# guzba/zippy

Hardware: NVIDIA H100
Metric: compress_level1_gzip_input_throughput (higher is better)
Workload: dtype u8

## Files before the change

zippy_b200/csrc/zb_deflate.cu:

```cuda
#include "zb_device.cuh"
#include "zb_kernels.h"
#include "zb_huff_warp.cuh"

#define LZ_THREADS (ZB_WARPS_PER_CHUNK * 32)
#define LZ_HASH_BITS 11
#define LZ_TABLE_ENTRIES (1 << LZ_HASH_BITS)
#define LZ_PRESEED 2048
#ifndef ZB_LZ1_RESOLVE_WINNER
#define ZB_LZ1_RESOLVE_WINNER 0
#endif
#define LZ_LANE_CAP 32

#define LZ_PIECE_BYTES ZB_REC_PIECE_BYTES
#define LZ_PHASES (ZB_SUB_BYTES / LZ_PIECE_BYTES)
#define LZ_PHASE_BYTES (ZB_CHUNK_BYTES / LZ_PHASES)
#define LZ_PHASE_HIST 1024
#define LZ_BATCH_LPW 2
#define LZ_BATCH_WINDOWS (32 / LZ_BATCH_LPW)
static_assert(LZ_PIECE_BYTES * ZB_WARPS_PER_CHUNK == LZ_PHASE_BYTES, "one piece per warp and phase");
static_assert(LZ_PIECE_BYTES / ZB_WINDOW % LZ_BATCH_WINDOWS == 0, "a batch of windows never straddles two pieces");

#define LZ_SM_DATA 0
#define LZ_SM_DATA_BYTES (LZ_PHASE_BYTES + LZ_PHASE_HIST + 64 + 384)
#define LZ_SM_TABLE (LZ_SM_DATA + LZ_SM_DATA_BYTES)
#define LZ_SM_TABLE_BYTES (ZB_WARPS_PER_CHUNK * LZ_TABLE_ENTRIES * 2)
#define LZ_SM_HIST (LZ_SM_TABLE + LZ_SM_TABLE_BYTES)
#define LZ_SM_HIST_BYTES (ZB_WARPS_PER_CHUNK * ZB_HIST_WORDS * 4)
#define LZ_SM_RING (LZ_SM_HIST + LZ_SM_HIST_BYTES)
#define LZ_SM_RING_BYTES (ZB_WARPS_PER_CHUNK * LZ_BATCH_WINDOWS * ZB_MATCH_SLOTS * 4)
#define LZ_SM_LMUL (LZ_SM_RING + LZ_SM_RING_BYTES)
#define LZ_LMUL_PIECE 33
#define LZ_LMUL_PQ 49
#define LZ_SM_LMUL_BYTES (56 * 4)
#define LZ_SM_PART (LZ_SM_LMUL + LZ_SM_LMUL_BYTES)
#define LZ_SM_PART_BYTES (ZB_WARPS_PER_CHUNK * 24)
#define LZ_SM_BAR (LZ_SM_PART + LZ_SM_PART_BYTES)
#define LZ_SM_TOTAL (LZ_SM_BAR + 16)
static_assert(LZ_TABLE_ENTRIES * 2 >= 4096, "a warp's table region must hold the CRC step table");
static_assert(3 * (LZ_SM_TOTAL + 1024) <= 233472, "three CTAs per SM");
static_assert(LZ_SM_PART % 8 == 0 && LZ_SM_TABLE % 16 == 0, "alignment");

__device__ __forceinline__ uint32_t lz_hash(uint32_t v) { return (v * 0x9E3779B1u) >> (32 - LZ_HASH_BITS); }
__device__ __forceinline__ uint32_t shl_clamp(uint32_t x, uint32_t n) {
  uint32_t r;
  asm("shl.b32 %0, %1, %2;" : "=r"(r) : "r"(x), "r"(n));
  return r;
}
__device__ __forceinline__ uint32_t low_mask(uint32_t n) { return shl_clamp(1u, n) - 1u; }

__device__ __forceinline__ uint32_t lz_final_rec(uint32_t mlen, uint32_t dist, int &lc, int &dc) {
  uint32_t le, de;
  lc = (int)zb_len_code_bf(mlen, le);
  dc = (int)zb_dist_code_bf(dist, de);
  return (uint32_t)lc | (le << 5) | ((uint32_t)dc << 10) | (de << 15);
}


__device__ __forceinline__ void lz_select(const uint8_t *data, uint32_t off0, uint32_t wb, uint32_t b1, uint32_t cur,
                                          uint32_t nvalid, uint32_t &m, uint32_t dist, uint32_t *ring_slot,
                                          uint32_t &sel, uint32_t &ism, uint32_t &endw) {
  const int lane = zb_lane();
  const uint32_t mm = __ballot_sync(ZB_FULL, m != 0);
  endw = 0;
  ism = 0;
  if (mm) {
    const uint32_t lbit = 1u << lane;
    const uint32_t endp = (uint32_t)lane + m;
    const uint32_t rest = shl_clamp(1u, endp) ? (mm >> endp) : 0u;
    uint32_t nc = rest ? endp + (uint32_t)(__ffs((int)rest) - 1) : 32u;
    uint32_t vis = 1u << (cur + (uint32_t)(__ffs((int)(mm >> cur)) - 1));
#pragma unroll
    for (int r = 0; r < 3; r++) {
      vis |= __reduce_or_sync(ZB_FULL, (vis & lbit) ? shl_clamp(1u, nc) : 0u);
      const uint32_t t = __shfl_sync(ZB_FULL, nc, (int)(nc & 31u));
      nc = nc < 32u ? t : 32u;
    }
    ism = vis;
    const int lastm = 31 - __clz((int)ism);
    const uint32_t cov = (ism & lbit) ? (low_mask(endp) & ~low_mask((uint32_t)lane)) : 0u;
    const uint32_t covered = __reduce_or_sync(ZB_FULL, cov);
    uint32_t mlast = __shfl_sync(ZB_FULL, m, lastm);
    if (mlast >= LZ_LANE_CAP) {
      const uint32_t md = __shfl_sync(ZB_FULL, dist, lastm);
      const uint32_t pos = wb + (uint32_t)lastm;
      const uint32_t off = off0 + pos + LZ_LANE_CAP + 8u * (uint32_t)lane;
      uint32_t x0 = zb_ld32_unaligned(data, off) ^ zb_ld32_unaligned(data, off - md);
      uint32_t x1 = zb_ld32_unaligned(data, off + 4) ^ zb_ld32_unaligned(data, off + 4 - md);
      uint32_t nm = x0 ? ((uint32_t)(__ffs((int)x0) - 1) >> 3) : 4u + (x1 ? ((uint32_t)(__ffs((int)x1) - 1) >> 3) : 4u);
      uint32_t stop = __ballot_sync(ZB_FULL, nm < 8u);
      if (stop) {
        int first = __ffs((int)stop) - 1;
        mlast = LZ_LANE_CAP + 8u * (uint32_t)first + __shfl_sync(ZB_FULL, nm, first);
      } else {
        mlast = LZ_LANE_CAP + 256u;
      }
      mlast = min(mlast, min((uint32_t)ZB_MAX_MATCH, b1 - pos));
      if (lane == lastm) m = mlast;
    }
    sel = ism | (~covered & ~low_mask(cur) & low_mask(nvalid));
    endw = (uint32_t)lastm + mlast;
    if (ism & lbit) {
      uint32_t rank = (uint32_t)__popc(ism & (lbit - 1u));
      ring_slot[rank] = (m - 3u) | ((dist - 1u) << 9);
    }
  } else {
    sel = low_mask(nvalid) & ~low_mask(cur);
  }
}

template <int LPW, bool LITS>
__device__ __forceinline__ void lz_batch_pass(const uint8_t *wdata, bool active, uint32_t ksel, uint32_t kism,
                                              const uint32_t *ring_win, uint32_t *whist, uint2 *gmask_w,
                                              uint32_t *grecs_piece, uint32_t &rec_base) {
  constexpr int NW = 32 / LPW;
  const uint32_t part = (uint32_t)zb_lane() / NW, wi = (uint32_t)zb_lane() % NW;
  if (active && part == 0) *gmask_w = make_uint2(ksel, kism);
  const uint32_t im = active ? kism : 0u;
  const uint32_t pm = (0xffffffffu >> (32 - 32 / LPW)) << (part * (32 / LPW));
  uint32_t s = (LITS && active) ? (ksel & ~kism & pm) : 0u;
  while (s) {
    const uint32_t bit = (uint32_t)(__ffs((int)s) - 1);
    s &= s - 1;
    const uint32_t sy = wdata[bit];
    atomicAdd(&whist[sy >> 1], 1u << ((sy & 1u) * 16u));
  }
  const uint32_t nmatch = (uint32_t)__popc(im);
  uint32_t incl = nmatch;
#pragma unroll
  for (int o = 1; o < NW; o <<= 1) {
    const uint32_t t = __shfl_up_sync(ZB_FULL, incl, o, NW);
    if (wi >= (uint32_t)o) incl += t;
  }
  uint32_t *grecs_w = grecs_piece + rec_base + incl - nmatch;
  rec_base += __shfl_sync(ZB_FULL, incl, NW - 1);
  for (uint32_t k = part; k < nmatch; k += LPW) {
    const uint32_t raw = ring_win[k];
    int lc, dc;
    const uint32_t fin = lz_final_rec((raw & 511u) + 3u, (raw >> 9) + 1u, lc, dc);
    grecs_w[k] = fin;
    const uint32_t s1 = 257u + (uint32_t)lc, s2 = (uint32_t)ZB_NUM_LITLEN + (uint32_t)dc;
    atomicAdd(&whist[s1 >> 1], 1u << ((s1 & 1u) * 16u));
    atomicAdd(&whist[s2 >> 1], 1u << ((s2 & 1u) * 16u));
  }
}

#ifndef ZB_LZ1_STAGE_CLOCKS
#define ZB_LZ1_STAGE_CLOCKS 0
#endif
enum { LZS_WAIT, LZS_CHECKSUM, LZS_SEED, LZS_PROBE, LZS_EXTEND, LZS_SELECT, LZS_BATCH, LZS_BARRIER, LZS_N };
#if ZB_LZ1_STAGE_CLOCKS
__device__ unsigned long long zb_lz1_stage_clk[LZS_N];
#define LZ_CLK_DECL                          \
  unsigned long long clk_acc[LZS_N] = {};    \
  long long clk_t = clock64();
#define LZ_CLK(s)                            \
  if (MODE == 1) {                           \
    const long long clk_n = clock64();       \
    clk_acc[s] += (unsigned long long)(clk_n - clk_t); \
    clk_t = clk_n;                           \
  }
#define LZ_CLK_PUBLISH()                                                                           \
  if (MODE == 1 && lane == 0) {                                                                    \
    _Pragma("unroll") for (int s_ = 0; s_ < LZS_N; s_++) atomicAdd(&zb_lz1_stage_clk[s_], clk_acc[s_]); \
  }
extern "C" int zb200_lz1_stage_clocks(unsigned long long *out) {
  unsigned long long zero[LZS_N] = {};
  if (cudaMemcpyFromSymbol(out, zb_lz1_stage_clk, sizeof(zero)) != cudaSuccess) return -1;
  return cudaMemcpyToSymbol(zb_lz1_stage_clk, zero, sizeof(zero)) == cudaSuccess ? 0 : -1;
}
#else
#define LZ_CLK_DECL
#define LZ_CLK(s)
#define LZ_CLK_PUBLISH()
#endif

template <int MODE, int CK>
__global__ void __launch_bounds__(LZ_THREADS, 3)
    k_lz(const uint8_t *__restrict__ src, const ZbChunkDesc *__restrict__ desc, uint2 *__restrict__ masks,
         uint32_t *__restrict__ recs, uint16_t *__restrict__ hist, ZbChunkCheck *__restrict__ chk,
         const ZbCrcTables *__restrict__ tabs) {
  extern __shared__ __align__(128) uint8_t smem[];
  uint8_t *data = smem + LZ_SM_DATA;
  uint16_t *table_all = reinterpret_cast<uint16_t *>(smem + LZ_SM_TABLE);
  uint32_t *hist_all = reinterpret_cast<uint32_t *>(smem + LZ_SM_HIST);
  uint32_t *ring_all = reinterpret_cast<uint32_t *>(smem + LZ_SM_RING);
  uint32_t *lane_mul = reinterpret_cast<uint32_t *>(smem + LZ_SM_LMUL);
  uint64_t *part = reinterpret_cast<uint64_t *>(smem + LZ_SM_PART);
  uint64_t *bar = reinterpret_cast<uint64_t *>(smem + LZ_SM_BAR);

  const uint32_t chunk = blockIdx.x;
  const ZbChunkDesc d = desc[chunk];
  const uint32_t len = d.len;
  const int tid = (int)threadIdx.x, lane = tid & 31;
  const int warp = (int)__reduce_max_sync(ZB_FULL, (uint32_t)tid >> 5);

  if (tid == 0) {
    zb_mbar_init(bar, 1);
    zb_fence_mbar_init();
  }
  __syncthreads();
  const uint32_t mis = (uint32_t)((uintptr_t)(src + d.src_off) & 15u);

  uint16_t *table = table_all + warp * LZ_TABLE_ENTRIES;
  uint32_t *ring = ring_all + warp * LZ_BATCH_WINDOWS * ZB_MATCH_SLOTS;
  uint2 *gmask = masks + (size_t)chunk * ZB_WINDOWS_PER_CHUNK;
  uint32_t acc_crc = 0;
  uint64_t acc_a = 0, acc_b = 0;
  LZ_CLK_DECL

  for (uint32_t ph = 0; ph < LZ_PHASES; ph++) {
    const uint32_t pbase = ph * LZ_PHASE_BYTES;
    if (ph && pbase >= len) break;
    const uint32_t sbase = ph ? pbase - LZ_PHASE_HIST : 0u;
    if (ph) __syncthreads();
    LZ_CLK(LZS_BARRIER)
    if (tid == 0 && len) {
      zb_fence_proxy_async();
      zb_stage_chunk(data, src + d.src_off + sbase, min(len, pbase + LZ_PHASE_BYTES + 384u) - sbase, bar);
    }
    if (CK & ZB_CK_CRC) {
      uint32_t *crc_tab = reinterpret_cast<uint32_t *>(table);
      for (int i = lane; i < 1024; i += 32) crc_tab[i] = (&tabs->mul1024[0][0])[i];
    }
    if (ph == 0) {
      for (int i = tid; i < ZB_WARPS_PER_CHUNK * ZB_HIST_WORDS; i += LZ_THREADS) hist_all[i] = 0;
      if (tid < 33) lane_mul[tid] = tabs->lane_mul[tid];
      if (tid >= 64 && tid < 80) lane_mul[LZ_LMUL_PIECE + tid - 64] = tabs->piece_mul[tid - 64];
      if (tid >= 96 && tid < 100) lane_mul[LZ_LMUL_PQ + tid - 96] = tabs->pq_mul[tid - 96];
      __syncthreads();
    } else {
      __syncwarp();
    }
    if (len) zb_mbar_wait(bar, ph & 1u);
    LZ_CLK(LZS_WAIT)

    const uint32_t b0 = pbase + (uint32_t)warp * LZ_PIECE_BYTES;
    if (b0 >= len) continue;
    const uint32_t b1 = min(b0 + LZ_PIECE_BYTES, len);
    const uint32_t doff = mis - sbase;
    uint32_t *whist = hist_all + (b0 / ZB_SUB_BYTES) * ZB_HIST_WORDS;

    if (CK) {
      ZbCheck c = zb_warp_checksums<LZ_PIECE_BYTES, LZ_LMUL_PQ, CK>(data, doff + b0, b1 - b0,
                                                                    reinterpret_cast<const uint32_t *>(table), lane_mul);
      const uint32_t after = len - b1;
      if (after) {
        if (CK & ZB_CK_CRC) {
          const uint32_t shift = ((after & (LZ_PIECE_BYTES - 1)) == 0) ? lane_mul[LZ_LMUL_PIECE + after / LZ_PIECE_BYTES]
                                                                       : zb_xpow8_t(tabs->pow2, after);
          c.crc_raw = zb_gf2_mul(c.crc_raw, shift);
        }
        if (CK & ZB_CK_ADLER) c.b_sum += (uint64_t)after * c.a_sum;
      }
      acc_crc ^= c.crc_raw;
      acc_a += c.a_sum;
      acc_b += c.b_sum;
      __syncwarp();
    }
    LZ_CLK(LZS_CHECKSUM)

    if (MODE == 1) {
      uint4 ff = make_uint4(~0u, ~0u, ~0u, ~0u);
      uint4 *t4 = reinterpret_cast<uint4 *>(table);
      for (int i = lane; i < LZ_TABLE_ENTRIES * 2 / 16; i += 32) t4[i] = ff;
      __syncwarp();
      for (uint32_t s = b0 - min((uint32_t)LZ_PRESEED, b0 - sbase); s < b0; s += 32) {
        const uint32_t p = s + (uint32_t)lane;
        const bool can = p + 4 <= len;
        const uint32_t h = lz_hash(zb_ld32_unaligned(data, doff + p));
        if (can) table[h] = (uint16_t)p;
#if ZB_LZ1_RESOLVE_WINNER
        __syncwarp();
        for (;;) {
          const bool lost = can && table[h] < (uint16_t)p;
          if (!__any_sync(ZB_FULL, lost)) break;
          if (lost) table[h] = (uint16_t)p;
          __syncwarp();
        }
#endif
      }
      __syncwarp();
    }
    LZ_CLK(LZS_SEED)
    uint32_t entry = b0;
    uint32_t ksel = 0, kism = 0;
    uint32_t *grecs = recs + (size_t)chunk * ZB_RECS_PER_CHUNK + (b0 >> 2);
    uint32_t rec_base = 0;
    const uint32_t bl = (uint32_t)lane & (LZ_BATCH_WINDOWS - 1u);
    for (uint32_t wb = b0; wb < b1; wb += 32) {
      const uint32_t win = wb >> 5, slot = win & (LZ_BATCH_WINDOWS - 1u);
      uint32_t sel = 0, ism = 0;
      if (entry < wb + 32) {
        const uint32_t p = wb + (uint32_t)lane;
        const uint32_t nvalid = min(32u, b1 - wb);
        const uint32_t cur = entry - wb;
        uint32_t m = 0, c = 0, lit = 0;
        if (MODE == 1) {
          const uint32_t *wp = reinterpret_cast<const uint32_t *>(data) + ((doff + p) >> 2);
          const uint32_t sp = ((doff + p) & 3u) * 8u;
          const uint32_t p0 = wp[0], p1 = wp[1];
          const uint32_t v = __funnelshift_r(p0, p1, sp);
          lit = v & 255u;
          const bool can = (p + 4 <= len);
          const uint32_t h = lz_hash(v);
          c = table[h];
          __syncwarp();
          if (can) table[h] = (uint16_t)p;
#if ZB_LZ1_RESOLVE_WINNER
          __syncwarp();
          for (;;) {
            const bool lost = can && table[h] < (uint16_t)p;
            if (!__any_sync(ZB_FULL, lost)) break;
            if (lost) table[h] = (uint16_t)p;
            __syncwarp();
          }
#endif
          LZ_CLK(LZS_PROBE)
          const uint32_t limit = p < b1 ? min((uint32_t)ZB_MAX_MATCH, b1 - p) : 0u;
          if (can && c < p && p - c <= ZB_MAX_DIST && p >= entry && limit >= ZB_MIN_MATCH) {
            const uint32_t *wc = reinterpret_cast<const uint32_t *>(data) + ((doff + c) >> 2);
            const uint32_t sc = ((doff + c) & 3u) * 8u;
            uint32_t hp = p1, hc = wc[1];
            uint32_t np = wp[2], nq = wc[2], np2 = wp[3], nq2 = wc[3];
            if (__funnelshift_r(wc[0], hc, sc) == v) {
              m = 4;
#pragma unroll 1
              for (int k = 2;; k += 2) {
                const uint32_t x = __funnelshift_r(hp, np, sp) ^ __funnelshift_r(hc, nq, sc);
                const uint32_t x2 = __funnelshift_r(np, np2, sp) ^ __funnelshift_r(nq, nq2, sc);
                if (x) {
                  m += (uint32_t)(__ffs((int)x) - 1) >> 3;
                  break;
                }
                if (k == LZ_LANE_CAP / 4) {
                  m += 4;
                  break;
                }
                if (x2) {
                  m += 4u + ((uint32_t)(__ffs((int)x2) - 1) >> 3);
                  break;
                }
                m += 8;
                hp = np2;
                hc = nq2;
                np = wp[k + 2];
                nq = wc[k + 2];
                np2 = wp[k + 3];
                nq2 = wc[k + 3];
              }
              if (m < LZ_LANE_CAP) m = min(m, limit);
            }
          }
          LZ_CLK(LZS_EXTEND)
        }
        uint32_t endw;
        lz_select(data, doff, wb, b1, cur, nvalid, m, p - c, ring + slot * ZB_MATCH_SLOTS, sel, ism, endw);
        entry = wb + max(endw, nvalid);
        if (MODE == 1 && ((sel & ~ism) >> lane & 1u)) atomicAdd(&whist[lit >> 1], 1u << ((lit & 1u) * 16u));
        LZ_CLK(LZS_SELECT)
      }
      if (bl == slot) {
        ksel = sel;
        kism = ism;
      }
      if (slot == LZ_BATCH_WINDOWS - 1u || wb + 32 >= b1) {
        __syncwarp();
        const uint32_t bwin = win - slot + bl;
        lz_batch_pass<LZ_BATCH_LPW, MODE != 1>(data + (uint32_t)(doff + (bwin << 5)), bl <= slot, ksel, kism, ring + bl * ZB_MATCH_SLOTS,
                                    whist, gmask + bwin, grecs, rec_base);
        ksel = kism = 0;
        __syncwarp();
      }
      LZ_CLK(LZS_BATCH)
    }
  }
  if (lane == 0) {
    part[warp * 3 + 0] = acc_crc;
    part[warp * 3 + 1] = acc_a;
    part[warp * 3 + 2] = acc_b;
  }
  __syncthreads();
  {
    uint32_t *gh = reinterpret_cast<uint32_t *>(hist + (size_t)chunk * ZB_WARPS_PER_CHUNK * ZB_HIST_SYMS);
    for (int i = tid; i < ZB_WARPS_PER_CHUNK * ZB_HIST_WORDS; i += LZ_THREADS) gh[i] = hist_all[i];
  }
  LZ_CLK(LZS_BARRIER)
  LZ_CLK_PUBLISH()
  if (tid == 0) {
    uint32_t raw = 0;
    uint64_t a = 0, b = 0;
    for (int w = 0; w < ZB_WARPS_PER_CHUNK; w++) {
      raw ^= (uint32_t)part[w * 3 + 0];
      a += part[w * 3 + 1];
      b += part[w * 3 + 2];
    }
    ZbChunkCheck cc;
    cc.crc_raw = raw;
    cc.adler = (CK & ZB_CK_ADLER) ? zb_adler_from_sums(a % ZB_ADLER_MOD, b % ZB_ADLER_MOD, len) : 0u;
    chk[chunk] = cc;
  }
}

#define LZ2_HIST 32768
#define LZ2_SEG_BYTES ZB_SUB_BYTES
#define LZ2_SEGS ((ZB_CHUNK_BYTES + LZ2_HIST) / LZ2_SEG_BYTES)
#define LZ2_BUCKET_BITS 11
#define LZ2_BUCKETS (1 << LZ2_BUCKET_BITS)
#define LZ2_TABLES_PER_CTA (ZB_WARPS_PER_CHUNK + LZ2_SEGS)
#define LZ2_RING_WINDOWS 8
#define LZ2_SM_DATA_BYTES (ZB_CHUNK_BYTES + LZ2_HIST + 64 + 384)
#define LZ2_SM_HIST (LZ2_SM_DATA_BYTES)
#define LZ2_SM_RING (LZ2_SM_HIST + LZ_SM_HIST_BYTES)
#define LZ2_SM_RING_BYTES (ZB_WARPS_PER_CHUNK * LZ2_RING_WINDOWS * ZB_MATCH_SLOTS * 4)
#define LZ2_SM_CRC (LZ2_SM_RING + LZ2_SM_RING_BYTES)
#define LZ2_SM_LMUL (LZ2_SM_CRC + 4096)
#define LZ2_SM_PART (LZ2_SM_LMUL + LZ_SM_LMUL_BYTES)
#define LZ2_SM_LIST (LZ2_SM_PART + LZ_SM_PART_BYTES)
#define LZ2_SM_BAR (LZ2_SM_LIST + 8 * LZ_THREADS * 2)
#define LZ2_SM_TOTAL (LZ2_SM_BAR + 16)
static_assert(2 * (LZ2_SM_TOTAL + 1024) <= 233472, "two CTAs per SM");

#ifndef LZ2_CTAS_PER_SM
#define LZ2_CTAS_PER_SM 1
#endif
#ifndef LZ2_STATIC_BITS
#define LZ2_STATIC_BITS 13
#endif
__device__ __forceinline__ uint32_t lz2_hash_mul(uint32_t v) { return v * 0x9E3779B1u; }
__device__ __forceinline__ uint32_t lz2_hash(uint32_t v) { return lz2_hash_mul(v) >> (32 - LZ2_BUCKET_BITS); }

__device__ __forceinline__ uint2 lz2_push(uint2 b, uint32_t e) {
  uint2 r;
  r.y = __funnelshift_l(b.x, b.y, 16);
  r.x = (b.x << 16) | (e & 0xffffu);
  return r;
}

__device__ __forceinline__ void lz2_clear_table(uint2 *tab, int bytes = LZ2_BUCKETS * 8) {
  const uint4 ff = make_uint4(~0u, ~0u, ~0u, ~0u);
  uint4 *t4 = reinterpret_cast<uint4 *>(tab);
  for (int i = zb_lane(); i < bytes / 16; i += 32) __stcg(&t4[i], ff);
}

__device__ __forceinline__ uint2 lz2_probe_insert(uint2 *tab, uint32_t h, bool can, uint32_t qwin, uint32_t &grp) {
  const int lane = zb_lane();
  grp = __match_any_sync(ZB_FULL, can ? h : (0x80000000u | (uint32_t)lane));
  uint2 old = make_uint2(~0u, ~0u);
  if (can) old = __ldcg(&tab[h]);
  __syncwarp();
  if (can && lane == 31 - __clz((int)grp)) {
    uint2 nb = old;
    for (uint32_t g = grp; g; g &= g - 1) nb = lz2_push(nb, qwin + (uint32_t)(__ffs((int)g) - 1));
    __stcg(&tab[h], nb);
  }
  __syncwarp();
  return old;
}

struct Lz2Pos {
  const uint32_t *data32;
  uint32_t poff;
  uint32_t q;
  uint32_t v;
  uint32_t lim;
  uint32_t limit, stop;
};

#define LZ2_LIST 8
__device__ __forceinline__ void lz2_verify(const Lz2Pos &P, uint32_t e, bool search, uint16_t *dl, uint32_t &n) {
  const uint32_t d = (P.q - e) & 0xffffu;
  if (!search || (d - 1u) >= P.lim) return;
  const uint32_t co = P.poff - d;
  const uint32_t *wc = P.data32 + (co >> 2);
  if (__funnelshift_r(wc[0], wc[1], (co & 3u) * 8u) != P.v) return;
// ... 764 lines not shown
    if (!cb->is_final) {
      nb += 3u;
      nb += (8u - ((pos + nb) & 7u)) & 7u;
      tv |= 0xffff0000ull << nb;
      nb += 32u;
    } else {
      nb += (8u - ((pos + nb) & 7u)) & 7u;
    }
    while (nb) {
      const uint32_t rel = pos >> 5, sh = pos & 31u, take = min(nb, 32u - sh);
      const uint32_t bits = (uint32_t)(tv & ((1ull << take) - 1ull)) << sh;
      if (sh == 0 && take == 32u) dstw_rel[rel] = bits;
      else pk_edge_or(&ed, rel, bits);
      tv >>= take;
      pos += take;
      nb -= take;
    }
  }
  __syncthreads();
  if (tid < PK_EDGES && ed.used[tid] && (tid == 0 || ed.word[tid] != ed.word[tid - 1])) {
    const uint32_t rel = ed.word[tid], val = ed.val[tid];
    const uint32_t lo = rel * 32u, hi = lo + 32u;
    if (lo >= B0 && hi <= end_bit) dstw_rel[rel] = val;
    else {
      uint8_t *bp = reinterpret_cast<uint8_t *>(dstw_rel + rel);
      for (uint32_t j = 0; j < 4; j++)
        if (lo + 8u * j >= B0 && lo + 8u * j + 8u <= end_bit) bp[j] = (uint8_t)(val >> (8u * j));
    }
  }
}

static bool zb_is_lz_level(int level) { return level == -1 || level >= 2; }
ZbLz2Params zb_lz2_params(int level) {
  static const ZbLz2Params table[10] = {{4, 4, 4, 8, 16}, {4, 4, 4, 8, 16}, {2, 4, 2, 4, 0},  {2, 4, 3, 4, 6},   {3, 4, 3, 4, 8},
                                        {3, 4, 4, 8, 16}, {4, 4, 4, 8, 16}, {4, 4, 6, 8, 32}, {4, 4, 8, 16, 32}, {4, 4, 8, 32, 64}};
  return table[(level >= 2 && level <= 9) ? level : 6];
}
size_t zb_lz2_table_bytes(int *grid_out) {
  int grid = LZ2_CTAS_PER_SM * zb_sm_count();
  if (grid_out) *grid_out = grid;
  return (size_t)grid * LZ2_TABLES_PER_CTA * LZ2_BUCKETS * sizeof(uint2);
}
typedef void (*ZbLzKernel)(const uint8_t *, const ZbChunkDesc *, uint2 *, uint32_t *, uint16_t *, ZbChunkCheck *,
                           const ZbCrcTables *);
static ZbLzKernel zb_lz_kernel(int mode, int data_format, bool index_crc = false) {
  if (index_crc && data_format == ZB_DF_ZLIB) return mode ? k_lz<1, ZB_CK_CRC | ZB_CK_ADLER> : k_lz<0, ZB_CK_CRC | ZB_CK_ADLER>;
  if (index_crc) data_format = ZB_DF_GZIP;
  const int ck = data_format == ZB_DF_GZIP ? ZB_CK_CRC : data_format == ZB_DF_ZLIB ? ZB_CK_ADLER : 0;
  if (mode) return ck == ZB_CK_CRC ? k_lz<1, ZB_CK_CRC> : ck == ZB_CK_ADLER ? k_lz<1, ZB_CK_ADLER> : k_lz<1, 0>;
  return ck == ZB_CK_CRC ? k_lz<0, ZB_CK_CRC> : ck == ZB_CK_ADLER ? k_lz<0, ZB_CK_ADLER> : k_lz<0, 0>;
}
cudaError_t zb_setup_deflate_attrs() {
  cudaError_t e = cudaSuccess;
  static const int fmts[3] = {ZB_DF_GZIP, ZB_DF_ZLIB, ZB_DF_DEFLATE};
  for (int mode = 0; mode < 2; mode++)
    for (int f = 0; f < 4; f++) {
      const ZbLzKernel k = f < 3 ? zb_lz_kernel(mode, fmts[f]) : zb_lz_kernel(mode, ZB_DF_ZLIB, true);
      if (e == cudaSuccess) e = cudaFuncSetAttribute(k, cudaFuncAttributeMaxDynamicSharedMemorySize, LZ_SM_TOTAL);
      if (e == cudaSuccess) e = cudaFuncSetAttribute(k, cudaFuncAttributePreferredSharedMemoryCarveout, cudaSharedmemCarveoutMaxShared);
    }
  if (e == cudaSuccess) e = cudaFuncSetAttribute(k_lz2<false>, cudaFuncAttributeMaxDynamicSharedMemorySize, LZ2_SM_TOTAL);
  if (e == cudaSuccess) e = cudaFuncSetAttribute(k_lz2<true>, cudaFuncAttributeMaxDynamicSharedMemorySize, LZ2_SM_TOTAL);
  cudaFuncAttributes fa;
  if (e == cudaSuccess) e = cudaFuncGetAttributes(&fa, k_huff);
  if (e == cudaSuccess) e = cudaFuncGetAttributes(&fa, k_scan);
  if (e == cudaSuccess) e = cudaFuncGetAttributes(&fa, k_member_check);
  if (e == cudaSuccess) e = cudaFuncGetAttributes(&fa, k_pack);
  if (e == cudaSuccess) e = cudaFuncGetAttributes(&fa, k_index_rec);
  return e;
}
cudaError_t zb_launch_lz(const ZbCompressWork &w, cudaStream_t s, bool index_crc) {
  if (w.n_chunks == 0) return cudaSuccess;
  if (zb_is_lz_level(w.level)) {
    int grid = 0;
    (void)zb_lz2_table_bytes(&grid);
    if ((uint32_t)grid > w.n_chunks) grid = (int)w.n_chunks;
    if (w.win16)
      k_lz2<true><<<grid, LZ_THREADS, LZ2_SM_TOTAL, s>>>(w.src, w.desc, w.masks, w.recs, w.hist, w.chk, w.tabs, w.lz2_tables,
                                                         w.n_chunks, zb_lz2_params(w.level), w.win16, w.win_len, w.win_stride);
    else
      k_lz2<false><<<grid, LZ_THREADS, LZ2_SM_TOTAL, s>>>(w.src, w.desc, w.masks, w.recs, w.hist, w.chk, w.tabs, w.lz2_tables,
                                                          w.n_chunks, zb_lz2_params(w.level), nullptr, 0u, 0u);
  } else {
    const ZbLzKernel k = zb_lz_kernel((w.level == -2 || w.level == 0) ? 0 : 1, w.data_format, index_crc);
    k<<<w.n_chunks, LZ_THREADS, LZ_SM_TOTAL, s>>>(w.src, w.desc, w.masks, w.recs, w.hist, w.chk, w.tabs);
  }
  return cudaGetLastError();
}
cudaError_t zb_launch_huff(const ZbCompressWork &w, cudaStream_t s) {
  if (w.n_chunks == 0) return cudaSuccess;
  k_huff<<<(w.n_chunks + HW_WARPS - 1) / HW_WARPS, HW_WARPS * 32, 0, s>>>(w.desc, w.hist, w.cb, w.n_chunks, w.level);
  return cudaGetLastError();
}
cudaError_t zb_launch_scan(const ZbCompressWork &w, cudaStream_t s) {
  k_scan<<<1, SCAN_THREADS, 0, s>>>(w);
  if (w.n_members) k_member_check<<<(w.n_members + 3) / 4, 128, 0, s>>>(w);
  return cudaGetLastError();
}
cudaError_t zb_launch_index_rec(const ZbCompressWork &w, const ZbIndexWork &x, cudaStream_t s) {
  if (w.n_chunks == 0) return cudaSuccess;
  k_index_rec<<<(w.n_chunks + 127) / 128, 128, 0, s>>>(w, x);
  return cudaGetLastError();
}
cudaError_t zb_launch_pack(const ZbCompressWork &w, cudaStream_t s) {
  if (w.n_chunks == 0) return cudaSuccess;
  k_pack<<<w.n_chunks, LZ_THREADS, 0, s>>>(w);
  return cudaGetLastError();
}
```

zippy_b200/csrc/zb_device.cuh:

```cuda
#pragma once
#include <cuda_runtime.h>
#include <stdint.h>

#include "zb_common.h"
#include "zb_crc.h"

#define ZB_FULL 0xffffffffu

static inline int zb_sm_count() {
  int dev = 0, sms = 132;
  cudaGetDevice(&dev);
  cudaDeviceGetAttribute(&sms, cudaDevAttrMultiProcessorCount, dev);
  return sms;
}

__device__ __forceinline__ uint32_t zb_smem_addr(const void *p) {
  return (uint32_t)__cvta_generic_to_shared(p);
}
__device__ __forceinline__ int zb_lane() { return (int)(threadIdx.x & 31u); }

__device__ __forceinline__ void zb_mbar_init(uint64_t *bar, uint32_t count) {
  asm volatile("mbarrier.init.shared::cta.b64 [%0], %1;" ::"r"(zb_smem_addr(bar)), "r"(count) : "memory");
}
__device__ __forceinline__ void zb_fence_proxy_async() { asm volatile("fence.proxy.async.shared::cta;" ::: "memory"); }
__device__ __forceinline__ void zb_fence_mbar_init() {
  asm volatile("fence.mbarrier_init.release.cluster;" ::: "memory");
}
__device__ __forceinline__ void zb_mbar_expect_tx(uint64_t *bar, uint32_t bytes) {
  asm volatile("mbarrier.arrive.expect_tx.shared::cta.b64 _, [%0], %1;" ::"r"(zb_smem_addr(bar)), "r"(bytes)
               : "memory");
}
__device__ __forceinline__ void zb_mbar_arrive(uint64_t *bar) {
  asm volatile("mbarrier.arrive.shared::cta.b64 _, [%0];" ::"r"(zb_smem_addr(bar)) : "memory");
}
__device__ __forceinline__ void zb_mbar_wait(uint64_t *bar, uint32_t parity) {
  asm volatile(
      "{\n"
      ".reg .pred p;\n"
      "ZB_WAIT_%=:\n"
      "mbarrier.try_wait.parity.shared::cta.b64 p, [%0], %1;\n"
      "@p bra ZB_DONE_%=;\n"
      "bra ZB_WAIT_%=;\n"
      "ZB_DONE_%=:\n"
      "}\n" ::"r"(zb_smem_addr(bar)),
      "r"(parity)
      : "memory");
}
__device__ __forceinline__ void zb_tma_load_1d(void *dst_smem, const void *src_gmem, uint32_t bytes,
                                               uint64_t *bar) {
  asm volatile(
      "cp.async.bulk.shared::cluster.global.mbarrier::complete_tx::bytes [%0], [%1], %2, [%3];" ::"r"(
          zb_smem_addr(dst_smem)),
      "l"(src_gmem), "r"(bytes), "r"(zb_smem_addr(bar))
      : "memory");
}

__device__ __forceinline__ uint32_t zb_stage_chunk(uint8_t *buf, const uint8_t *src, uint32_t len,
                                                   uint64_t *bar) {
  uint32_t mis = (uint32_t)((uintptr_t)src & 15u);
  uint32_t bytes = (mis + len + 15u) & ~15u;
  if (bytes == 0) bytes = 16;
  zb_mbar_expect_tx(bar, bytes);
  const uint8_t *g = src - mis;
  uint32_t done = 0;
  while (done < bytes) {
    uint32_t n = bytes - done;
    if (n > 32768u) n = 32768u;
    zb_tma_load_1d(buf + done, g + done, n, bar);
    done += n;
  }
  return mis;
}

__device__ __forceinline__ uint32_t zb_ld32_unaligned(const uint8_t *base, uint32_t off) {
  const uint32_t *w = reinterpret_cast<const uint32_t *>(base) + (off >> 2);
  uint32_t lo = w[0], hi = w[1];
  return __funnelshift_r(lo, hi, (off & 3u) * 8u);
}

__device__ __forceinline__ uint32_t zb_warp_xor(uint32_t v) {
#pragma unroll
  for (int o = 16; o > 0; o >>= 1) v ^= __shfl_xor_sync(ZB_FULL, v, o);
  return v;
}
__device__ __forceinline__ uint64_t zb_warp_sum64(uint64_t v) {
#pragma unroll
  for (int o = 16; o > 0; o >>= 1) v += __shfl_xor_sync(ZB_FULL, v, o);
  return v;
}

__device__ __forceinline__ uint32_t zb_mul1024(const uint32_t *tab , uint32_t r, uint32_t ts = 1u) {
  return tab[(r & 255u) * ts] ^ tab[(256 + ((r >> 8) & 255u)) * ts] ^ tab[(512 + ((r >> 16) & 255u)) * ts] ^ tab[(768 + (r >> 24)) * ts];
}

struct ZbCheck {
  uint32_t crc_raw;
  uint64_t a_sum, b_sum;
};
#define ZB_CK_CRC 1
#define ZB_CK_ADLER 2
template <uint32_t FULL = ZB_SUB_BYTES, int QOFF = 41, int WANT = ZB_CK_CRC | ZB_CK_ADLER>
__device__ __forceinline__ ZbCheck zb_warp_checksums(const uint8_t *base, uint32_t off, uint32_t n,
                                                     const uint32_t *tab, const uint32_t *lane_mul, uint32_t ts = 1u) {
  const int lane = zb_lane();
  if (ts != 1u) tab += lane;
  if (n == FULL && ts == 1u) {
    uint32_t r0 = 0, r1 = 0, r2 = 0, r3 = 0, a = 0;
    uint64_t b = 0;
    const uint32_t o = off + 4u * (uint32_t)lane, rel0 = 4u * (uint32_t)lane;
    constexpr uint32_t QR = FULL / 512;
    constexpr uint32_t QB = FULL / 4;
#pragma unroll 2
    for (uint32_t k = 0; k < QR; k++) {
      const uint32_t w0 = zb_ld32_unaligned(base, o + 128u * k), w1 = zb_ld32_unaligned(base, o + 128u * (QR + k));
      const uint32_t w2 = zb_ld32_unaligned(base, o + 128u * (2u * QR + k)), w3 = zb_ld32_unaligned(base, o + 128u * (3u * QR + k));
      if (WANT & ZB_CK_CRC) {
        if (k) {
          r0 = zb_mul1024(tab, r0);
          r1 = zb_mul1024(tab, r1);
          r2 = zb_mul1024(tab, r2);
          r3 = zb_mul1024(tab, r3);
        }
        r0 ^= w0;
        r1 ^= w1;
        r2 ^= w2;
        r3 ^= w3;
      }
      if (!(WANT & ZB_CK_ADLER)) continue;
      const uint32_t s0 = __dp4a(w0, 0x01010101u, 0u), s1 = __dp4a(w1, 0x01010101u, 0u);
      const uint32_t s2 = __dp4a(w2, 0x01010101u, 0u), s3 = __dp4a(w3, 0x01010101u, 0u);
      a += s0 + s1 + s2 + s3;
      const uint32_t rel = rel0 + 128u * k;
      b += (uint64_t)(4u * QB - rel) * s0 + (uint64_t)(3u * QB - rel) * s1 + (uint64_t)(2u * QB - rel) * s2 +
           (uint64_t)(QB - rel) * s3;
      b -= (uint64_t)(__dp4a(w0, 0x03020100u, 0u) + __dp4a(w1, 0x03020100u, 0u) + __dp4a(w2, 0x03020100u, 0u) +
                      __dp4a(w3, 0x03020100u, 0u));
    }
    ZbCheck out;
    out.crc_raw = 0;
    out.a_sum = out.b_sum = 0;
    if (WANT & ZB_CK_CRC) {
      uint32_t r = zb_gf2_mul(r0, lane_mul[QOFF + 3]) ^ zb_gf2_mul(r1, lane_mul[QOFF + 2]) ^ zb_gf2_mul(r2, lane_mul[QOFF + 1]) ^ r3;
      r = zb_gf2_mul(r, lane_mul[32 - lane]);
      out.crc_raw = zb_warp_xor(r);
    }
    if (WANT & ZB_CK_ADLER) {
      out.a_sum = zb_warp_sum64((uint64_t)a);
      out.b_sum = zb_warp_sum64(b);
    }
    return out;
  }
  const uint32_t rows = n >> 7, tail = n & 127u;
  uint32_t r = 0;
  uint32_t a = 0;
  uint64_t b = 0;
  uint32_t o = off + 4u * (uint32_t)lane;
  uint32_t rel = 4u * (uint32_t)lane;
  for (uint32_t k = 0; k < rows; k++) {
    uint32_t w = zb_ld32_unaligned(base, o);
    if (k) r = zb_mul1024(tab, r, ts);
    r ^= w;
    uint32_t s = __dp4a(w, 0x01010101u, 0u);
    uint32_t ws = __dp4a(w, 0x03020100u, 0u);
    a += s;
    b += (uint64_t)(n - rel) * s - ws;
    o += 128u;
    rel += 128u;
  }
  uint32_t crc = rows ? zb_gf2_mul(r, lane_mul[32 - lane]) : 0u;
  const uint32_t tw = tail >> 2, rem = tail & 3u;
  uint32_t crc_tail = 0;
  if ((uint32_t)lane < tw) {
    uint32_t w = zb_ld32_unaligned(base, o);
    crc_tail = zb_gf2_mul(w, lane_mul[tw - (uint32_t)lane]);
    uint32_t s = __dp4a(w, 0x01010101u, 0u);
    uint32_t ws = __dp4a(w, 0x03020100u, 0u);
    a += s;
    b += (uint64_t)(n - rel) * s - ws;
  }
  uint32_t crc_rem = 0;
  if (lane == 0) {
    for (uint32_t i = 0; i < rem; i++) {
      uint32_t byte = base[off + (rows << 7) + 4u * tw + i];
      crc_rem = zb_crc_raw_byte(crc_rem, byte);
      a += byte;
      b += (uint64_t)(rem - i) * byte;
    }
  }
  ZbCheck out;
  out.crc_raw = 0;
  out.a_sum = out.b_sum = 0;
  if (WANT & ZB_CK_CRC) {
    crc = zb_warp_xor(crc);
    crc_tail = zb_warp_xor(crc_tail);
    crc_rem = __shfl_sync(ZB_FULL, crc_rem, 0);
    uint32_t raw = crc;
    if (tail) {
      raw = zb_gf2_mul(crc, zb_xpow8(tail));
      if (rem) raw ^= zb_gf2_mul(crc_tail, zb_xpow8(rem)) ^ crc_rem;
      else raw ^= crc_tail;
    }
    out.crc_raw = raw;
  }
  if (WANT & ZB_CK_ADLER) {
    out.a_sum = zb_warp_sum64((uint64_t)a);
    out.b_sum = zb_warp_sum64(b);
  }
  return out;
}
```

Baseline: 80.83.

## Offload level-1 checksums to dedicated extra warps in the LZ kernel

New measurement: 80.99 (median of 6 runs). No clear change (+0.2%).

```diff
diff --git a/zippy_b200/csrc/zb_deflate.cu b/zippy_b200/csrc/zb_deflate.cu
--- a/zippy_b200/csrc/zb_deflate.cu
+++ b/zippy_b200/csrc/zb_deflate.cu
@@ -174,8 +174,16 @@
 #define LZ_CLK_PUBLISH()
 #endif
 
+#define LZ_CK_WARPS 4
+static_assert(ZB_WARPS_PER_CHUNK % LZ_CK_WARPS == 0, "every checksum warp takes the same number of pieces");
 template <int MODE, int CK>
-__global__ void __launch_bounds__(LZ_THREADS, 3)
+struct LzThreads {
+  static constexpr bool split = MODE == 1 && CK != 0;
+  static constexpr int value = LZ_THREADS + (split ? LZ_CK_WARPS * 32 : 0);
+};
+
+template <int MODE, int CK>
+__global__ void __launch_bounds__(LzThreads<MODE, CK>::value, 3)
     k_lz(const uint8_t *__restrict__ src, const ZbChunkDesc *__restrict__ desc, uint2 *__restrict__ masks,
          uint32_t *__restrict__ recs, uint16_t *__restrict__ hist, ZbChunkCheck *__restrict__ chk,
          const ZbCrcTables *__restrict__ tabs) {
@@ -193,6 +201,8 @@
   const uint32_t len = d.len;
   const int tid = (int)threadIdx.x, lane = tid & 31;
   const int warp = (int)__reduce_max_sync(ZB_FULL, (uint32_t)tid >> 5);
+  constexpr bool SPLIT = LzThreads<MODE, CK>::split;
+  constexpr int NT = LzThreads<MODE, CK>::value;
 
   if (tid == 0) {
     zb_mbar_init(bar, 1);
@@ -218,12 +228,17 @@
       zb_fence_proxy_async();
       zb_stage_chunk(data, src + d.src_off + sbase, min(len, pbase + LZ_PHASE_BYTES + 384u) - sbase, bar);
     }
-    if (CK & ZB_CK_CRC) {
+    if (SPLIT) {
+      if (warp < ZB_WARPS_PER_CHUNK) {
+        uint4 *t4 = reinterpret_cast<uint4 *>(table);
+        for (int i = lane; i < LZ_TABLE_ENTRIES * 2 / 16; i += 32) t4[i] = make_uint4(~0u, ~0u, ~0u, ~0u);
+      }
+    } else if (CK & ZB_CK_CRC) {
       uint32_t *crc_tab = reinterpret_cast<uint32_t *>(table);
       for (int i = lane; i < 1024; i += 32) crc_tab[i] = (&tabs->mul1024[0][0])[i];
     }
     if (ph == 0) {
-      for (int i = tid; i < ZB_WARPS_PER_CHUNK * ZB_HIST_WORDS; i += LZ_THREADS) hist_all[i] = 0;
+      for (int i = tid; i < ZB_WARPS_PER_CHUNK * ZB_HIST_WORDS; i += NT) hist_all[i] = 0;
       if (tid < 33) lane_mul[tid] = tabs->lane_mul[tid];
       if (tid >= 64 && tid < 80) lane_mul[LZ_LMUL_PIECE + tid - 64] = tabs->piece_mul[tid - 64];
       if (tid >= 96 && tid < 100) lane_mul[LZ_LMUL_PQ + tid - 96] = tabs->pq_mul[tid - 96];
@@ -234,13 +249,38 @@
     if (len) zb_mbar_wait(bar, ph & 1u);
     LZ_CLK(LZS_WAIT)
 
+    if (SPLIT && warp >= ZB_WARPS_PER_CHUNK) {
+      const uint32_t doff = mis - sbase;
+      for (uint32_t q = (uint32_t)(warp - ZB_WARPS_PER_CHUNK); q < ZB_WARPS_PER_CHUNK; q += LZ_CK_WARPS) {
+        const uint32_t b0 = pbase + q * LZ_PIECE_BYTES;
+        if (b0 >= len) break;
+        const uint32_t b1 = min(b0 + LZ_PIECE_BYTES, len);
+        ZbCheck c = zb_warp_checksums<LZ_PIECE_BYTES, LZ_LMUL_PQ, CK>(data, doff + b0, b1 - b0, &tabs->mul1024[0][0],
+                                                                      lane_mul);
+        const uint32_t after = len - b1;
+        if (after) {
+          if (CK & ZB_CK_CRC) {
+            const uint32_t shift = ((after & (LZ_PIECE_BYTES - 1)) == 0) ? lane_mul[LZ_LMUL_PIECE + after / LZ_PIECE_BYTES]
+                                                                         : zb_xpow8_t(tabs->pow2, after);
+            c.crc_raw = zb_gf2_mul(c.crc_raw, shift);
+          }
+          if (CK & ZB_CK_ADLER) c.b_sum += (uint64_t)after * c.a_sum;
+        }
+        acc_crc ^= c.crc_raw;
+        acc_a += c.a_sum;
+        acc_b += c.b_sum;
+      }
+      LZ_CLK(LZS_CHECKSUM)
+      continue;
+    }
+
     const uint32_t b0 = pbase + (uint32_t)warp * LZ_PIECE_BYTES;
     if (b0 >= len) continue;
     const uint32_t b1 = min(b0 + LZ_PIECE_BYTES, len);
     const uint32_t doff = mis - sbase;
     uint32_t *whist = hist_all + (b0 / ZB_SUB_BYTES) * ZB_HIST_WORDS;
 
-    if (CK) {
+    if (CK && !SPLIT) {
       ZbCheck c = zb_warp_checksums<LZ_PIECE_BYTES, LZ_LMUL_PQ, CK>(data, doff + b0, b1 - b0,
                                                                     reinterpret_cast<const uint32_t *>(table), lane_mul);
       const uint32_t after = len - b1;
@@ -260,9 +300,11 @@
     LZ_CLK(LZS_CHECKSUM)
 
     if (MODE == 1) {
-      uint4 ff = make_uint4(~0u, ~0u, ~0u, ~0u);
-      uint4 *t4 = reinterpret_cast<uint4 *>(table);
-      for (int i = lane; i < LZ_TABLE_ENTRIES * 2 / 16; i += 32) t4[i] = ff;
+      if (!SPLIT) {
+        uint4 ff = make_uint4(~0u, ~0u, ~0u, ~0u);
+        uint4 *t4 = reinterpret_cast<uint4 *>(table);
+        for (int i = lane; i < LZ_TABLE_ENTRIES * 2 / 16; i += 32) t4[i] = ff;
+      }
       __syncwarp();
       for (uint32_t s = b0 - min((uint32_t)LZ_PRESEED, b0 - sbase); s < b0; s += 32) {
         const uint32_t p = s + (uint32_t)lane;
@@ -374,22 +416,23 @@
       LZ_CLK(LZS_BATCH)
     }
   }
-  if (lane == 0) {
-    part[warp * 3 + 0] = acc_crc;
-    part[warp * 3 + 1] = acc_a;
-    part[warp * 3 + 2] = acc_b;
+  const int pslot = SPLIT ? warp - ZB_WARPS_PER_CHUNK : warp;
+  if (lane == 0 && pslot >= 0) {
+    part[pslot * 3 + 0] = acc_crc;
+    part[pslot * 3 + 1] = acc_a;
+    part[pslot * 3 + 2] = acc_b;
   }
   __syncthreads();
   {
     uint32_t *gh = reinterpret_cast<uint32_t *>(hist + (size_t)chunk * ZB_WARPS_PER_CHUNK * ZB_HIST_SYMS);
-    for (int i = tid; i < ZB_WARPS_PER_CHUNK * ZB_HIST_WORDS; i += LZ_THREADS) gh[i] = hist_all[i];
+    for (int i = tid; i < ZB_WARPS_PER_CHUNK * ZB_HIST_WORDS; i += NT) gh[i] = hist_all[i];
   }
   LZ_CLK(LZS_BARRIER)
   LZ_CLK_PUBLISH()
   if (tid == 0) {
     uint32_t raw = 0;
     uint64_t a = 0, b = 0;
-    for (int w = 0; w < ZB_WARPS_PER_CHUNK; w++) {
+    for (int w = 0; w < (SPLIT ? LZ_CK_WARPS : ZB_WARPS_PER_CHUNK); w++) {
       raw ^= (uint32_t)part[w * 3 + 0];
       a += part[w * 3 + 1];
       b += part[w * 3 + 2];
@@ -1320,8 +1363,11 @@
       k_lz2<false><<<grid, LZ_THREADS, LZ2_SM_TOTAL, s>>>(w.src, w.desc, w.masks, w.recs, w.hist, w.chk, w.tabs, w.lz2_tables,
                                                           w.n_chunks, zb_lz2_params(w.level), nullptr, 0u, 0u);
   } else {
-    const ZbLzKernel k = zb_lz_kernel((w.level == -2 || w.level == 0) ? 0 : 1, w.data_format, index_crc);
-    k<<<w.n_chunks, LZ_THREADS, LZ_SM_TOTAL, s>>>(w.src, w.desc, w.masks, w.recs, w.hist, w.chk, w.tabs);
+    const int mode = (w.level == -2 || w.level == 0) ? 0 : 1;
+    const ZbLzKernel k = zb_lz_kernel(mode, w.data_format, index_crc);
+    const bool split = mode && (index_crc || w.data_format == ZB_DF_GZIP || w.data_format == ZB_DF_ZLIB);
+    k<<<w.n_chunks, split ? LzThreads<1, ZB_CK_CRC>::value : LZ_THREADS, LZ_SM_TOTAL, s>>>(w.src, w.desc, w.masks,
+                                                                                        w.recs, w.hist, w.chk, w.tabs);
   }
   return cudaGetLastError();
 }
```

## Use nibble CRC tables, batch hash preseed loads, and restructure level-1 match batching

Applied to the files above, without the earlier changes.

Result: faster. 80.64 before, 82.55 after, median of 6 (+2.4%).

```diff
diff --git a/zippy_b200/csrc/zb_deflate.cu b/zippy_b200/csrc/zb_deflate.cu
--- a/zippy_b200/csrc/zb_deflate.cu
+++ b/zippy_b200/csrc/zb_deflate.cu
@@ -17,8 +17,15 @@
 #define LZ_PHASE_HIST 1024
 #define LZ_BATCH_LPW 2
 #define LZ_BATCH_WINDOWS (32 / LZ_BATCH_LPW)
+#define LZ_RING_SLOTS (LZ_BATCH_WINDOWS * ZB_MATCH_SLOTS)
+#ifndef LZ1_BATCH_WINDOWS
+#define LZ1_BATCH_WINDOWS 32
+#endif
 static_assert(LZ_PIECE_BYTES * ZB_WARPS_PER_CHUNK == LZ_PHASE_BYTES, "one piece per warp and phase");
 static_assert(LZ_PIECE_BYTES / ZB_WINDOW % LZ_BATCH_WINDOWS == 0, "a batch of windows never straddles two pieces");
+static_assert(LZ_PIECE_BYTES / ZB_WINDOW % LZ1_BATCH_WINDOWS == 0 && LZ1_BATCH_WINDOWS <= 32, "k_lz<1>'s batches too");
+static_assert(LZ_PRESEED % (8 * ZB_WINDOW) == 0 && LZ_PHASE_HIST % (8 * ZB_WINDOW) == 0 && LZ_PIECE_BYTES % (8 * ZB_WINDOW) == 0,
+              "a pre-seed is a whole number of groups of eight rows");
 
 #define LZ_SM_DATA 0
 #define LZ_SM_DATA_BYTES (LZ_PHASE_BYTES + LZ_PHASE_HIST + 64 + 384)
@@ -27,7 +34,7 @@
 #define LZ_SM_HIST (LZ_SM_TABLE + LZ_SM_TABLE_BYTES)
 #define LZ_SM_HIST_BYTES (ZB_WARPS_PER_CHUNK * ZB_HIST_WORDS * 4)
 #define LZ_SM_RING (LZ_SM_HIST + LZ_SM_HIST_BYTES)
-#define LZ_SM_RING_BYTES (ZB_WARPS_PER_CHUNK * LZ_BATCH_WINDOWS * ZB_MATCH_SLOTS * 4)
+#define LZ_SM_RING_BYTES (ZB_WARPS_PER_CHUNK * LZ_RING_SLOTS * 4)
 #define LZ_SM_LMUL (LZ_SM_RING + LZ_SM_RING_BYTES)
 #define LZ_LMUL_PIECE 33
 #define LZ_LMUL_PQ 49
@@ -36,7 +43,7 @@
 #define LZ_SM_PART_BYTES (ZB_WARPS_PER_CHUNK * 24)
 #define LZ_SM_BAR (LZ_SM_PART + LZ_SM_PART_BYTES)
 #define LZ_SM_TOTAL (LZ_SM_BAR + 16)
-static_assert(LZ_TABLE_ENTRIES * 2 >= 4096, "a warp's table region must hold the CRC step table");
+static_assert(LZ_TABLE_ENTRIES * 2 >= 512, "a warp's table region must hold the CRC step tables");
 static_assert(3 * (LZ_SM_TOTAL + 1024) <= 233472, "three CTAs per SM");
 static_assert(LZ_SM_PART % 8 == 0 && LZ_SM_TABLE % 16 == 0, "alignment");
 
@@ -144,6 +151,17 @@
   }
 }
 
+__device__ __forceinline__ void lz1_batch_recs(const uint32_t *ring, uint32_t n, uint32_t *whist, uint32_t *grecs_b) {
+  for (uint32_t j = (uint32_t)zb_lane(); j < n; j += 32) {
+    const uint32_t raw = ring[j];
+    int lc, dc;
+    grecs_b[j] = lz_final_rec((raw & 511u) + 3u, (raw >> 9) + 1u, lc, dc);
+    const uint32_t s1 = 257u + (uint32_t)lc, s2 = (uint32_t)ZB_NUM_LITLEN + (uint32_t)dc;
+    atomicAdd(&whist[s1 >> 1], 1u << ((s1 & 1u) * 16u));
+    atomicAdd(&whist[s2 >> 1], 1u << ((s2 & 1u) * 16u));
+  }
+}
+
 #ifndef ZB_LZ1_STAGE_CLOCKS
 #define ZB_LZ1_STAGE_CLOCKS 0
 #endif
@@ -202,10 +220,11 @@
   const uint32_t mis = (uint32_t)((uintptr_t)(src + d.src_off) & 15u);
 
   uint16_t *table = table_all + warp * LZ_TABLE_ENTRIES;
-  uint32_t *ring = ring_all + warp * LZ_BATCH_WINDOWS * ZB_MATCH_SLOTS;
+  uint32_t *ring = ring_all + warp * LZ_RING_SLOTS;
   uint2 *gmask = masks + (size_t)chunk * ZB_WINDOWS_PER_CHUNK;
   uint32_t acc_crc = 0;
   uint64_t acc_a = 0, acc_b = 0;
+  constexpr uint32_t BW = MODE == 1 ? LZ1_BATCH_WINDOWS : LZ_BATCH_WINDOWS;
   LZ_CLK_DECL
 
   for (uint32_t ph = 0; ph < LZ_PHASES; ph++) {
@@ -220,7 +239,14 @@
     }
     if (CK & ZB_CK_CRC) {
       uint32_t *crc_tab = reinterpret_cast<uint32_t *>(table);
-      for (int i = lane; i < 1024; i += 32) crc_tab[i] = (&tabs->mul1024[0][0])[i];
+      uint32_t v[4];
+#pragma unroll
+      for (int q = 0; q < 4; q++) {
+        const uint32_t i = (uint32_t)lane + 32u * (uint32_t)q, j = i >> 4;
+        v[q] = tabs->mul1024[j >> 1][(i & 15u) << (4u * (j & 1u))];
+      }
+#pragma unroll
+      for (int q = 0; q < 4; q++) crc_tab[lane + 32 * q] = v[q];
     }
     if (ph == 0) {
       for (int i = tid; i < ZB_WARPS_PER_CHUNK * ZB_HIST_WORDS; i += LZ_THREADS) hist_all[i] = 0;
@@ -241,7 +267,7 @@
     uint32_t *whist = hist_all + (b0 / ZB_SUB_BYTES) * ZB_HIST_WORDS;
 
     if (CK) {
-      ZbCheck c = zb_warp_checksums<LZ_PIECE_BYTES, LZ_LMUL_PQ, CK>(data, doff + b0, b1 - b0,
+      ZbCheck c = zb_warp_checksums<LZ_PIECE_BYTES, LZ_LMUL_PQ, CK, true>(data, doff + b0, b1 - b0,
                                                                     reinterpret_cast<const uint32_t *>(table), lane_mul);
       const uint32_t after = len - b1;
       if (after) {
@@ -264,20 +290,26 @@
       uint4 *t4 = reinterpret_cast<uint4 *>(table);
       for (int i = lane; i < LZ_TABLE_ENTRIES * 2 / 16; i += 32) t4[i] = ff;
       __syncwarp();
-      for (uint32_t s = b0 - min((uint32_t)LZ_PRESEED, b0 - sbase); s < b0; s += 32) {
-        const uint32_t p = s + (uint32_t)lane;
-        const bool can = p + 4 <= len;
-        const uint32_t h = lz_hash(zb_ld32_unaligned(data, doff + p));
-        if (can) table[h] = (uint16_t)p;
+      for (uint32_t s = b0 - min((uint32_t)LZ_PRESEED, b0 - sbase); s < b0; s += 8 * 32) {
+        uint32_t v[8];
+#pragma unroll
+        for (int k = 0; k < 8; k++) v[k] = zb_ld32_unaligned(data, doff + s + 32u * (uint32_t)k + (uint32_t)lane);
+#pragma unroll
+        for (int k = 0; k < 8; k++) {
+          const uint32_t p = s + 32u * (uint32_t)k + (uint32_t)lane;
+          const bool can = p + 4 <= len;
+          const uint32_t h = lz_hash(v[k]);
+          if (can) table[h] = (uint16_t)p;
 #if ZB_LZ1_RESOLVE_WINNER
-        __syncwarp();
-        for (;;) {
-          const bool lost = can && table[h] < (uint16_t)p;
-          if (!__any_sync(ZB_FULL, lost)) break;
-          if (lost) table[h] = (uint16_t)p;
           __syncwarp();
-        }
+          for (;;) {
+            const bool lost = can && table[h] < (uint16_t)p;
+            if (!__any_sync(ZB_FULL, lost)) break;
+            if (lost) table[h] = (uint16_t)p;
+            __syncwarp();
+          }
 #endif
+        }
       }
       __syncwarp();
     }
@@ -286,9 +318,11 @@
     uint32_t ksel = 0, kism = 0;
     uint32_t *grecs = recs + (size_t)chunk * ZB_RECS_PER_CHUNK + (b0 >> 2);
     uint32_t rec_base = 0;
-    const uint32_t bl = (uint32_t)lane & (LZ_BATCH_WINDOWS - 1u);
+    uint32_t rb = 0;
+    uint32_t bs = 0;
+    const uint32_t bl = (uint32_t)lane & (BW - 1u);
     for (uint32_t wb = b0; wb < b1; wb += 32) {
-      const uint32_t win = wb >> 5, slot = win & (LZ_BATCH_WINDOWS - 1u);
+      const uint32_t win = wb >> 5, slot = win & (BW - 1u);
       uint32_t sel = 0, ism = 0;
       if (entry < wb + 32) {
         const uint32_t p = wb + (uint32_t)lane;
@@ -354,7 +388,8 @@
           LZ_CLK(LZS_EXTEND)
         }
         uint32_t endw;
-        lz_select(data, doff, wb, b1, cur, nvalid, m, p - c, ring + slot * ZB_MATCH_SLOTS, sel, ism, endw);
+        lz_select(data, doff, wb, b1, cur, nvalid, m, p - c, MODE == 1 ? ring + rb : ring + slot * ZB_MATCH_SLOTS, sel,
+                  ism, endw);
         entry = wb + max(endw, nvalid);
         if (MODE == 1 && ((sel & ~ism) >> lane & 1u)) atomicAdd(&whist[lit >> 1], 1u << ((lit & 1u) * 16u));
         LZ_CLK(LZS_SELECT)
@@ -363,7 +398,19 @@
         ksel = sel;
         kism = ism;
       }
-      if (slot == LZ_BATCH_WINDOWS - 1u || wb + 32 >= b1) {
+      if (MODE == 1) {
+        rb += (uint32_t)__popc(ism);
+        if (slot == BW - 1u || wb + 32 >= b1 || (BW * ZB_MATCH_SLOTS > LZ_RING_SLOTS && rb > LZ_RING_SLOTS - ZB_MATCH_SLOTS)) {
+          __syncwarp();
+          if ((uint32_t)lane < BW && bl >= bs && bl <= slot) gmask[win - slot + bl] = make_uint2(ksel, kism);
+          lz1_batch_recs(ring, rb, whist, grecs + rec_base);
+          rec_base += rb;
+          rb = 0;
+          bs = (slot + 1u) & (BW - 1u);
+          ksel = kism = 0;
+          __syncwarp();
+        }
+      } else if (slot == LZ_BATCH_WINDOWS - 1u || wb + 32 >= b1) {
         __syncwarp();
         const uint32_t bwin = win - slot + bl;
         lz_batch_pass<LZ_BATCH_LPW, MODE != 1>(data + (uint32_t)(doff + (bwin << 5)), bl <= slot, ksel, kism, ring + bl * ZB_MATCH_SLOTS,
diff --git a/zippy_b200/csrc/zb_device.cuh b/zippy_b200/csrc/zb_device.cuh
--- a/zippy_b200/csrc/zb_device.cuh
+++ b/zippy_b200/csrc/zb_device.cuh
@@ -93,13 +93,20 @@
   return tab[(r & 255u) * ts] ^ tab[(256 + ((r >> 8) & 255u)) * ts] ^ tab[(512 + ((r >> 16) & 255u)) * ts] ^ tab[(768 + (r >> 24)) * ts];
 }
 
+__device__ __forceinline__ uint32_t zb_mul1024_nib(const uint32_t *tab , uint32_t r) {
+  uint32_t x = 0;
+#pragma unroll
+  for (int j = 0; j < 8; j++) x ^= tab[16 * j + ((r >> (4 * j)) & 15u)];
+  return x;
+}
+
 struct ZbCheck {
   uint32_t crc_raw;
   uint64_t a_sum, b_sum;
 };
 #define ZB_CK_CRC 1
 #define ZB_CK_ADLER 2
-template <uint32_t FULL = ZB_SUB_BYTES, int QOFF = 41, int WANT = ZB_CK_CRC | ZB_CK_ADLER>
+template <uint32_t FULL = ZB_SUB_BYTES, int QOFF = 41, int WANT = ZB_CK_CRC | ZB_CK_ADLER, bool NIB = false>
 __device__ __forceinline__ ZbCheck zb_warp_checksums(const uint8_t *base, uint32_t off, uint32_t n,
                                                      const uint32_t *tab, const uint32_t *lane_mul, uint32_t ts = 1u) {
   const int lane = zb_lane();
@@ -116,10 +123,10 @@
       const uint32_t w2 = zb_ld32_unaligned(base, o + 128u * (2u * QR + k)), w3 = zb_ld32_unaligned(base, o + 128u * (3u * QR + k));
       if (WANT & ZB_CK_CRC) {
         if (k) {
-          r0 = zb_mul1024(tab, r0);
-          r1 = zb_mul1024(tab, r1);
-          r2 = zb_mul1024(tab, r2);
-          r3 = zb_mul1024(tab, r3);
+          r0 = NIB ? zb_mul1024_nib(tab, r0) : zb_mul1024(tab, r0);
+          r1 = NIB ? zb_mul1024_nib(tab, r1) : zb_mul1024(tab, r1);
+          r2 = NIB ? zb_mul1024_nib(tab, r2) : zb_mul1024(tab, r2);
+          r3 = NIB ? zb_mul1024_nib(tab, r3) : zb_mul1024(tab, r3);
         }
         r0 ^= w0;
         r1 ^= w1;
@@ -158,7 +165,7 @@
   uint32_t rel = 4u * (uint32_t)lane;
   for (uint32_t k = 0; k < rows; k++) {
     uint32_t w = zb_ld32_unaligned(base, o);
-    if (k) r = zb_mul1024(tab, r, ts);
+    if (k) r = NIB ? zb_mul1024_nib(tab, r) : zb_mul1024(tab, r, ts);
     r ^= w;
     uint32_t s = __dp4a(w, 0x01010101u, 0u);
     uint32_t ws = __dp4a(w, 0x03020100u, 0u);
```
